# Hfx-J/SGTD

Hardware: AMD Instinct MI355X
Metric: query frames/sec vs map size (descriptor build + candidate selection) (higher is better)
Workload: dtype f64

## Files before the change

### sgtd_amd/csrc/build_kernel.hip.h

```cpp
#pragma once
#include "common.hip.h"

struct DescArrays {
  double *side, *angle, *center;
  float *vertex;
  int *label;
  u32 *frame;
  int *node_id;
  QueryRec *qrec;
};

#define SGTD_BUILD_THREADS 1024
#ifdef SGTD_EXP_PHASE
__device__ unsigned long long g_bphase[8];
#define BPH(i) do { if (tid == 0) { const unsigned long long _n = __builtin_readcyclecounter(); atomicAdd(&g_bphase[i], _n - bph_t); bph_t = _n; } } while (0)
#else
#define BPH(i) do { } while (0)
#endif
#define SGTD_TRI_INVALID 0xFFFFFFFFFFFFFFFFull
#define SGTD_SLOT_EMPTY 0xFFFFFFFFu

struct Tri {
  double a, b, c;
  int va, vb, vc;
  bool valid;
};

__device__ __forceinline__ double side_len(const float4 &p, const float4 &q) {
  double dx = (double)(p.x - q.x), dy = (double)(p.y - q.y), dz = (double)(p.z - q.z);
  return sqrt(dx * dx + dy * dy + dz * dz);
}

__device__ __forceinline__ Tri make_triangle(const float4 &p1, const float4 &p2,
                                             const float4 &p3, const DevCfg &cfg) {
  Tri t;
  double a = side_len(p1, p2), b = side_len(p1, p3), c = side_len(p3, p2);
  t.valid = !(a > cfg.max_len || b > cfg.max_len || c > cfg.max_len ||
              a < cfg.min_len || b < cfg.min_len || c < cfg.min_len);
  int sa = 0, sb = 1, sc = 2;
  double tmp; int ti;
  if (a > b) { tmp = a; a = b; b = tmp; ti = sa; sa = sb; sb = ti; }
  if (b > c) { tmp = b; b = c; c = tmp; ti = sb; sb = sc; sc = ti; }
  if (a > b) { tmp = a; a = b; b = tmp; ti = sa; sa = sb; sb = ti; }
  t.a = a; t.b = b; t.c = c;
  t.va = sa + sb - 1;
  t.vb = sa + sc - 1;
  t.vc = sb + sc - 1;
  return t;
}

__host__ __device__ __forceinline__ u64 pack_milli_key(u64 x, u64 y, u64 z) { return (x << 42) | (y << 21) | z; }
__device__ __forceinline__ u64 milli_key(const Tri &t) {
  float kx = (float)(t.a * 1000.0), ky = (float)(t.b * 1000.0), kz = (float)(t.c * 1000.0);
  u64 x = (u64)(long long)kx, y = (u64)(long long)ky, z = (u64)(long long)kz;
  return pack_milli_key(x, y, z);
}

struct BuildParams {
  const float *xyz;
  const u32 *label;
  const long long *kp_off;
  int n_frames;
  u32 frame_id0;
  int frame_id_step;
  long long out_stride;
  u32 *out_count;
  int max_n;
  int max_slots;
  u64 *ws_keys;
  u32 *ws_slots;
};

template <bool LDS_DEDUP, int KM>
__global__ __launch_bounds__(SGTD_BUILD_THREADS) void build_frames_kernel(
    BuildParams P, DevCfg cfg, DescArrays out) {
  extern __shared__ __align__(16) unsigned char smem[];
  const int K = cfg.K, tpi = cfg.tpi;
  const int max_t = P.max_n * tpi;
  const int max_words = (max_t + 31) / 32;
  float4 *pts = reinterpret_cast<float4 *>(smem);
  size_t off = (size_t)P.max_n * 16;
  unsigned short *knn = reinterpret_cast<unsigned short *>(smem + off);
  off += (((size_t)P.max_n * K * 2) + 15) & ~(size_t)15;
  unsigned char *mn = smem + off;
  off += (((size_t)tpi * 2) + 15) & ~(size_t)15;
  u32 *winbits = reinterpret_cast<u32 *>(smem + off);
  off += (((size_t)max_words * 4) + 15) & ~(size_t)15;
  u32 *wordpre = reinterpret_cast<u32 *>(smem + off);
  off += (((size_t)(max_words + 1) * 4) + 15) & ~(size_t)15;
  u64 *keys;
  u32 *slots;
  if (LDS_DEDUP) {
    keys = reinterpret_cast<u64 *>(smem + off);
    off += (size_t)max_t * 8;
    slots = reinterpret_cast<u32 *>(smem + off);
  } else {
    keys = P.ws_keys + (size_t)blockIdx.x * max_t;
    slots = P.ws_slots + (size_t)blockIdx.x * P.max_slots;
  }
  const int tid = threadIdx.x;

  if (tid == 0) {
    int k = 0;
    for (int m = 1; m < K - 1; m++)
      for (int n = m + 1; n < K; n++) {
        mn[2 * k] = (unsigned char)m;
        mn[2 * k + 1] = (unsigned char)n;
        k++;
      }
  }

  for (int f = blockIdx.x; f < P.n_frames; f += gridDim.x) {
    const long long kp0 = P.kp_off[f];
    const int n = (int)(P.kp_off[f + 1] - kp0);
    __syncthreads();
    if (n < K) {
      if (tid == 0) P.out_count[f] = 0;
      continue;
    }
    const int T = n * tpi;
    int nslots = 64;
    while (nslots < T + 1) nslots <<= 1;
    const int nwords = (T + 31) / 32;

#ifdef SGTD_EXP_PHASE
    unsigned long long bph_t = __builtin_readcyclecounter();
#endif
    for (int i = tid; i < n; i += SGTD_BUILD_THREADS) {
      float4 p;
      p.x = P.xyz[(kp0 + i) * 3 + 0];
      p.y = P.xyz[(kp0 + i) * 3 + 1];
      p.z = P.xyz[(kp0 + i) * 3 + 2];
      p.w = __uint_as_float(P.label[kp0 + i]);
      pts[i] = p;
    }
    for (int s = tid; s < nslots; s += SGTD_BUILD_THREADS) slots[s] = SGTD_SLOT_EMPTY;
    for (int w = tid; w < nwords; w += SGTD_BUILD_THREADS) winbits[w] = 0;
    __syncthreads();

    BPH(0);
    const int parts = (3 * K <= tpi) ? 4 : 1;
    const int per_pass = SGTD_BUILD_THREADS / parts;
    for (int i0 = 0; i0 < n; i0 += per_pass) {
      const int i = i0 + tid / parts, part = tid % parts;
      float bd[KM];
      int bi[KM];
#pragma unroll
      for (int k = 0; k < KM; k++) { bd[k] = __builtin_inff(); bi[k] = 0; }
      auto insert = [&](float cd, int cj) {
        bool lt = false;
#pragma unroll
        for (int k = 0; k < KM; k++) {
          lt = lt || (cd < bd[k]);
          float td = lt ? bd[k] : cd; int tj = lt ? bi[k] : cj;
          bd[k] = lt ? cd : bd[k]; bi[k] = lt ? cj : bi[k];
          cd = td; cj = tj;
        }
      };
      if (i < n) {
        const float4 q = pts[i];
        const int j_lo = (int)((long long)n * part / parts), j_hi = (int)((long long)n * (part + 1) / parts);
        for (int j = j_lo; j < j_hi; j++) {
          const float4 p = pts[j];
          float dx = q.x - p.x, dy = q.y - p.y, dz = q.z - p.z;
          float d = dx * dx;
          d += dy * dy;
          d += dz * dz;
          insert(d, j);
        }
        if (part > 0) {
#pragma unroll
          for (int k = 0; k < KM; k++)
            if (k < K) keys[((size_t)i * 3 + (part - 1)) * K + k] = ((u64)__float_as_uint(bd[k]) << 32) | (u32)bi[k];
        }
      }
      if (parts > 1) {
        if (!LDS_DEDUP) __threadfence_block();
        __syncthreads();
        if (i < n && part == 0) {
          for (int pk = 0; pk < 3 * K; pk++) {
            const u64 v = keys[(size_t)i * 3 * K + pk];
            insert(__uint_as_float((u32)(v >> 32)), (int)(u32)v);
          }
        }
      }
      if (i < n && part == 0) {
#pragma unroll
        for (int k = 0; k < KM; k++)
          if (k < K) knn[i * K + k] = (unsigned short)bi[k];
      }
      if (parts > 1) __syncthreads();
    }
    __syncthreads();

    BPH(1);
    for (int t = tid; t < T; t += SGTD_BUILD_THREADS) {
      const int i = t / tpi, r = t - i * tpi;
      const int m = mn[2 * r], nn = mn[2 * r + 1];
      Tri tr = make_triangle(pts[i], pts[knn[i * K + m]], pts[knn[i * K + nn]], cfg);
      keys[t] = tr.valid ? milli_key(tr) : SGTD_TRI_INVALID;
    }
    if (!LDS_DEDUP) __threadfence_block();
    __syncthreads();

    BPH(2);
    for (int t = tid; t < T; t += SGTD_BUILD_THREADS) {
      const u64 key = keys[t];
      if (key == SGTD_TRI_INVALID) continue;
      u32 h = (u32)mix64(key) & (u32)(nslots - 1);
      while (true) {
        u32 cur = atomicCAS(&slots[h], SGTD_SLOT_EMPTY, (u32)t);
        if (cur == SGTD_SLOT_EMPTY) break;
        if (keys[cur] == key) { atomicMin(&slots[h], (u32)t); break; }
        h = (h + 1) & (u32)(nslots - 1);
      }
    }
    __syncthreads();
    for (int s = tid; s < nslots; s += SGTD_BUILD_THREADS) {
      u32 v = slots[s];
      if (v != SGTD_SLOT_EMPTY) atomicOr(&winbits[v >> 5], 1u << (v & 31));
    }
    __syncthreads();
    if (tid < SGTD_WAVE) {
      u32 carry = 0;
      for (int w0 = 0; w0 < nwords; w0 += SGTD_WAVE) {
        int w = w0 + tid;
        u32 c = (w < nwords) ? __popc(winbits[w]) : 0;
        u32 inc = wave_incl_scan(c);
        if (w < nwords) wordpre[w] = carry + inc - c;
        carry += __shfl(inc, SGTD_WAVE - 1);
      }
      if (tid == 0) { wordpre[nwords] = carry; P.out_count[f] = carry; }
    }
    __syncthreads();

    BPH(3);
    const u32 frame_id = P.frame_id0 + (u32)(P.frame_id_step * f);
    for (int t = tid; t < T; t += SGTD_BUILD_THREADS) {
      const u32 word = winbits[t >> 5];
      if (!((word >> (t & 31)) & 1u)) continue;
      const u32 rank = wordpre[t >> 5] + __popc(word & ((1u << (t & 31)) - 1u));
      const int i = t / tpi, r = t - i * tpi;
      const int m = mn[2 * r], nn = mn[2 * r + 1];
      float4 p[3];
      p[0] = pts[i]; p[1] = pts[knn[i * K + m]]; p[2] = pts[knn[i * K + nn]];
      const Tri tr = make_triangle(p[0], p[1], p[2], cfg);
      const float4 A = tr.va == 0 ? p[0] : (tr.va == 1 ? p[1] : p[2]);
      const float4 B = tr.vb == 0 ? p[0] : (tr.vb == 1 ? p[1] : p[2]);
      const float4 C = tr.vc == 0 ? p[0] : (tr.vc == 1 ? p[1] : p[2]);
      const size_t o = (size_t)f * P.out_stride + rank;
      const double a = tr.a, b = tr.b, c = tr.c;
      out.side[o * 3 + 0] = cfg.scale * a;
      out.side[o * 3 + 1] = cfg.scale * b;
      out.side[o * 3 + 2] = cfg.scale * c;
      out.angle[o * 3 + 0] = fabs((b * b + c * c - a * a) / (2 * b * c));
      out.angle[o * 3 + 1] = fabs((a * a + c * c - b * b) / (2 * a * c));
      out.angle[o * 3 + 2] = fabs((a * a + b * b - c * c) / (2 * a * b));
      out.center[o * 3 + 0] = (((double)A.x + (double)B.x) + (double)C.x) / 3;
      out.center[o * 3 + 1] = (((double)A.y + (double)B.y) + (double)C.y) / 3;
      out.center[o * 3 + 2] = (((double)A.z + (double)B.z) + (double)C.z) / 3;
      out.vertex[o * 9 + 0] = A.x; out.vertex[o * 9 + 1] = A.y; out.vertex[o * 9 + 2] = A.z;
      out.vertex[o * 9 + 3] = B.x; out.vertex[o * 9 + 4] = B.y; out.vertex[o * 9 + 5] = B.z;
      out.vertex[o * 9 + 6] = C.x; out.vertex[o * 9 + 7] = C.y; out.vertex[o * 9 + 8] = C.z;
      out.label[o * 3 + 0] = (int)(double)__float_as_uint(A.w);
      out.label[o * 3 + 1] = (int)(double)__float_as_uint(B.w);
      out.label[o * 3 + 2] = (int)(double)__float_as_uint(C.w);
      out.frame[o] = frame_id;
      if (out.qrec) write_query_rec(out.qrec + o, cfg.scale * a, cfg.scale * b, cfg.scale * c, cfg.rough, frame_id);
      out.node_id[o * 3 + 0] = i; out.node_id[o * 3 + 1] = m; out.node_id[o * 3 + 2] = nn;
    }
#ifdef SGTD_EXP_PHASE
    __syncthreads();
    BPH(4);
#endif
  }
}

static inline size_t build_lds_bytes(int max_n, int K, int tpi, bool lds_dedup, int max_slots) {
  size_t max_t = (size_t)max_n * tpi, words = (max_t + 31) / 32;
  auto up = [](size_t v) { return (v + 15) & ~(size_t)15; };
  size_t b = (size_t)max_n * 16 + up((size_t)max_n * K * 2) + up((size_t)tpi * 2) +
             up(words * 4) + up((words + 1) * 4);
  if (lds_dedup) b += max_t * 8 + (size_t)max_slots * 4;
  return b;
}
```

### sgtd_amd/csrc/sgtd_accel.hip

```cpp
#include "../../include/sgtd_accel.h"

#include <hip/hip_runtime.h>

#include <algorithm>
#include <atomic>
#include <chrono>
#include <cmath>
#include <cstdio>
#include <cstring>
#include <limits>
#include <memory>
#include <string>
#include <vector>

#include "build_kernel.hip.h"
#include "common.hip.h"
#include "table_kernels.hip.h"
#include "probe_kernels.hip.h"
#include "select_kernels.hip.h"
#include "verify_kernels.hip.h"
#include "verify_mfma.hip.h"
#include "exchange_kernels.hip.h"
#include "remove_kernels.hip.h"
#include "filter_kernels.hip.h"
// ... 114 lines not shown
  };
  Segment seg[2];
  int n_seg = 1;
  u32 append_min_frame = 0xFFFFFFFFu;
  int64_t tail_max = 0;
  float ms_finalize = 0.f;
  u32 coarse_at = 62, whole_at = 62;
  long long thr2_pending = 0;
  u32 rec_rate_hook = 0;
  u32 rec_rate_cap = 256;
  bool wide_pairs = false;
  int tail_batches = 0;
  DevBuf slice_of, sq_sum;
  DevBuf frame_first, by_frame, id_of_g, longest;
  u32 id_bits = 0;
  bool id_by_frame = false;
  DevBuf rm_bits, rm_present, rm_mask, rm_count, rm_scratch;
  std::shared_ptr<const FrameFilter> filt, batch_filt;
  DevBuf filt_rows;
  std::vector<u64> filt_host;
  u64 filt_rows_serial = 0;
  u32 filt_rows_lo = 0, filt_rows_span = 0;
  std::vector<float> poses;
  std::vector<unsigned char> has_pose;
  u64 poses_serial = 0;
  std::shared_ptr<const PositionPrior> prior, batch_prior;
  DevBuf pos_dev, prior_dev, filt_base;
  std::vector<float4> pos_host;
  u64 pos_serial = 0;
  u32 pos_lo = 0, pos_span = 0;
  u64 filt_base_serial = 0;
  u32 filt_base_lo = 0, filt_base_span = 0;
  struct PriorKey {
    u64 prior = 0, poses = 0, filt = 0;
    u32 lo = 0, span = 0;
    int n_rows = 0;
    bool operator==(const PriorKey &o) const { return prior == o.prior && poses == o.poses && filt == o.filt && lo == o.lo && span == o.span && n_rows == o.n_rows; }
  } prior_key;
  bool prior_rows_valid = false;
  DevBuf keyA, keyB, valA, valB, hist, digit_tot, flags, bad_flag;
  std::vector<DevBuf> scan_lvl;

  DevBuf kp_off_dev, xyz_dev, label_dev, ws_keys, ws_slots, cnt_scan;
  DevBuf b_kp_off_dev, b_xyz_dev, b_label_dev;
  DescStore tmp;
  DescStore fetch;
  DevBuf fetch_idx;
  DevBuf tmp_count;

  DescStore qd;
  DevBuf q_count;
  long long q_stride = 0;
  int nq = 0;
  bool batch_valid = false, batch_synced = false;
  int last_kind = 0;
  const float *last_xyz = nullptr;
  const u32 *last_label = nullptr;
  std::vector<long long> last_kp_off;
  int last_max_n = 0;
  u32 last_qframe = 0;
  bool loop_batch = false;
  int loop_skip = 0;
  DevBuf totals;
  DevBuf cursors, list, n_visit, votes, slot_of;
  DevBuf q_M, q_P, q_pairs, q_pair_base, blk_count, rec, rec_cell, rec_dis;
  DevBuf c_pair, c_blk;
  DevBuf amb_queue;
  DevBuf n_cand, cand_frame, cand_votes, pair_off, pairs;
  DevBuf v_score, v_pose, v_inlier, v_best;
  DevBuf inl_pairs, inl_off;
  bool verify_counted = false;
  DevBuf inl_counts;
  DevBuf in_block;
  size_t frame_inl_cap = 0;
  char *frame_host = nullptr;
  size_t frame_host_bytes = 0;
  DevBuf b_in, b_out;
  char *pin_build = nullptr;
  size_t pin_build_cap = 0;
  DevBuf v_hyp64, v_hyp32, v_bound;
  DevBuf v_hypB, v_tau, v_words;
  DevBuf v_okey[2], v_oval[2];
  bool verified = false;
  DevBuf r_pose, r_rmse, r_rmse_v, r_npairs, r_moments, r_flag;
  bool refined = false;
  int *export_packed = nullptr;
  size_t export_cap = 0;
  hipEvent_t ev_cand = nullptr, ev_export_free = nullptr;
  bool export_busy = false;
  u32 batch_serial = 0;
  bool defer_lists = false;
  bool lists_pending = false;
  bool lists_masked = false;
  bool fused_votes_last = false;
  const u64 *verify_keep = nullptr;
  const u64 *list_keep = nullptr;
  bool pairs_per_query = false;
  DevBuf rough_qi, rough_entry, rough_frame, rough_cell, rough_dis;
  size_t rec_cap = (size_t)1 << 25;
  bool rec_cap_fixed = false;
  size_t pair_cap = (size_t)1 << 24;
  DevBuf n_valid, cell_rows, gid, q_prefix, group_first, n_groups;
  DevBuf pos_of_slot, rec_off, pass_pool;
  size_t pool_units = 0;
  size_t group_cap = 0;
  size_t group_cap_hook = 0;
  int sorted_chunk = 0;
  bool diag = false;
  int select_mode = 0;
  PinnedVec<u32> h_count, h_pair_base, h_q_M;
  PinnedVec<unsigned long long> h_q_P;
  PinnedVec<int> h_n_cand, h_cand_frame, h_cand_votes;
  PinnedVec<long long> h_pair_off;
  sgtd_stats stats{};
  char *pin = nullptr;
  size_t pin_cap = 0, pin_used = 0;
  struct PinCopy { void *dst; size_t off, bytes; };
  std::vector<PinCopy> pin_pending;
};

#include "multi.hip.h"

namespace {

#define HIPCHK(call)                                                          \
  do {                                                                        \
    hipError_t _s = (call);                                                   \
    if (_s != hipSuccess) {                                                   \
      e->err = std::string(#call) + ": " + hipGetErrorString(_s);             \
      return SGTD_ERR_HIP;                                                    \
    }                                                                         \
  } while (0)
#define CHK(call)                 \
  do {                            \
    int _r = (call);              \
    if (_r != SGTD_OK) return _r; \
  } while (0)

int ensure(sgtd_engine *e, DevBuf &b, size_t bytes, bool keep = false) {
  if (bytes <= b.bytes) return SGTD_OK;
  if (b.borrowed) { e->err = "a table attached from another handle cannot grow here"; return SGTD_ERR_STATE; }
  size_t want = keep ? std::max(bytes, b.bytes + b.bytes / 2) : (b.p ? bytes + bytes / 4 : bytes);
  if (!keep && b.p) {
    HIPCHK(hipStreamSynchronize(e->stream));
    HIPCHK(hipFree(b.p));
    b.p = nullptr; b.bytes = 0;
  }
  void *np = nullptr;
  {
    const hipError_t st_ = hipMalloc(&np, want);
    if (st_ != hipSuccess) {
      (void)hipGetLastError();
      e->err = "hipMalloc of " + std::to_string(want) + " bytes: " + hipGetErrorString(st_);
      return SGTD_ERR_HIP;
    }
  }
  e->stats.device_allocs_total++;
  if (keep && b.p && b.bytes) {
    HIPCHK(hipMemcpyAsync(np, b.p, b.bytes, hipMemcpyDeviceToDevice, e->stream));
    HIPCHK(hipStreamSynchronize(e->stream));
  }
  if (b.p) HIPCHK(hipFree(b.p));
  b.p = np;
  b.bytes = want;
  return SGTD_OK;
}

int ensure_store(sgtd_engine *e, DescStore &s, size_t cap, bool keep = false) {
  if (cap <= s.cap) return SGTD_OK;
  size_t want = keep ? std::max(cap, s.cap + s.cap / 2) : cap;
  CHK(ensure(e, s.side, want * 3 * sizeof(double), keep));
  CHK(ensure(e, s.angle, want * 3 * sizeof(double), keep));
  CHK(ensure(e, s.center, want * 3 * sizeof(double), keep));
  CHK(ensure(e, s.vertex, want * 9 * sizeof(float), keep));
  CHK(ensure(e, s.label, want * 3 * sizeof(int), keep));
  CHK(ensure(e, s.frame, want * sizeof(u32), keep));
  CHK(ensure(e, s.node_id, want * 3 * sizeof(int), keep));
  if (s.with_thr2) CHK(ensure(e, s.qrec, want * sizeof(QueryRec), keep));
  s.cap = want;
  return SGTD_OK;
}

void free_buf(DevBuf &b) {
  if (b.p && !b.borrowed) (void)hipFree(b.p);
  b.p = nullptr;
  b.bytes = 0;
  b.borrowed = false;
}
void free_store(DescStore &s) {
  free_buf(s.side); free_buf(s.angle); free_buf(s.center); free_buf(s.vertex);
  free_buf(s.label); free_buf(s.frame); free_buf(s.node_id); free_buf(s.qrec);
  s.cap = 0;
}

constexpr size_t kPinMax = (size_t)1 << 20, kPinCap = (size_t)16 << 20;

int xfer_sync(sgtd_engine *e) {
  HIPCHK(hipStreamSynchronize(e->stream));
  for (const auto &c : e->pin_pending) std::memcpy(c.dst, e->pin + c.off, c.bytes);
  e->pin_pending.clear();
  e->pin_used = 0;
  return SGTD_OK;
}

struct PinScope {
  sgtd_engine *e;
  explicit PinScope(sgtd_engine *e_) : e(e_) {}
  ~PinScope() {
    if (e && !e->pin_pending.empty()) {
      (void)hipStreamSynchronize(e->stream);
      e->pin_pending.clear();
      e->pin_used = 0;
    }
  }
};

int pin_room(sgtd_engine *e, size_t bytes, size_t *off) {
  if (!e->pin) {
    void *p = nullptr;
    HIPCHK(hipHostMalloc(&p, kPinCap, hipHostMallocDefault));
    e->pin = static_cast<char *>(p);
    e->pin_cap = kPinCap;
  }
  const size_t need = (bytes + 255) & ~(size_t)255;
  if (e->pin_used + need > e->pin_cap) CHK(xfer_sync(e));
  *off = e->pin_used;
  e->pin_used += need;
  return SGTD_OK;
}

int d2h(sgtd_engine *e, void *dst, const void *src_dev, size_t bytes) {
  if (bytes == 0) return SGTD_OK;
  if (bytes > kPinMax) {
    HIPCHK(hipMemcpyAsync(dst, src_dev, bytes, hipMemcpyDeviceToHost, e->stream));
    return SGTD_OK;
  }
  size_t off;
  CHK(pin_room(e, bytes, &off));
  HIPCHK(hipMemcpyAsync(e->pin + off, src_dev, bytes, hipMemcpyDeviceToHost, e->stream));
  e->pin_pending.push_back({dst, off, bytes});
  return SGTD_OK;
}

int h2d(sgtd_engine *e, void *dst_dev, const void *src, size_t bytes) {
  if (bytes == 0) return SGTD_OK;
  if (bytes > kPinMax) {
    HIPCHK(hipMemcpyAsync(dst_dev, src, bytes, hipMemcpyHostToDevice, e->stream));
    return SGTD_OK;
  }
  size_t off;
  CHK(pin_room(e, bytes, &off));
  std::memcpy(e->pin + off, src, bytes);
  HIPCHK(hipMemcpyAsync(dst_dev, e->pin + off, bytes, hipMemcpyHostToDevice, e->stream));
  return SGTD_OK;
}

int grid_for(long long n, int threads) { return (int)((n + threads - 1) / threads); }
constexpr size_t kIndexLimit = 0xFFFFFFF0ull;
constexpr size_t kRecLimit = kIndexLimit << SGTD_REC_SHIFT;
template <class K>
size_t lds_room(K *kernel) {
  hipFuncAttributes a;
  const size_t fixed = hipFuncGetAttributes(&a, reinterpret_cast<const void *>(kernel)) == hipSuccess ? a.sharedSizeBytes : 16384;
  return std::min<size_t>(150 * 1024, 160 * 1024 - std::min<size_t>(fixed, 160 * 1024));
}

int device_scan(sgtd_engine *e, const u32 *in, u32 *out, long long n, size_t lvl = 0) {
  if (n <= 0) return SGTD_OK;
  const long long per = (long long)SGTD_SCAN_THREADS * SGTD_SCAN_ITEMS;
  const long long nb = (n + per - 1) / per;
  if (nb == 1) {
    scan_apply_kernel<<<1, SGTD_SCAN_THREADS, 0, e->stream>>>(in, out, nullptr, n);
    HIPCHK(hipGetLastError());
    return SGTD_OK;
  }
  if (e->scan_lvl.size() <= lvl) e->scan_lvl.resize(lvl + 1);
  CHK(ensure(e, e->scan_lvl[lvl], (size_t)nb * sizeof(u32)));
  u32 *sums = e->scan_lvl[lvl].as<u32>();
  scan_reduce_kernel<<<(int)nb, SGTD_SCAN_THREADS, 0, e->stream>>>(in, sums, n);
  HIPCHK(hipGetLastError());
  CHK(device_scan(e, sums, sums, nb, lvl + 1));
  sums = e->scan_lvl[lvl].as<u32>();
  scan_apply_kernel<<<(int)nb, SGTD_SCAN_THREADS, 0, e->stream>>>(in, out, sums, n);
  HIPCHK(hipGetLastError());
  return SGTD_OK;
}

int launch_build(sgtd_engine *e, const float *d_xyz, const u32 *d_label, const long long *d_kp_off,
                 int n_frames, int max_n, u32 frame_id0, int frame_step, DescArrays out,
                 long long out_stride, u32 *out_count) {
  if (n_frames <= 0) return SGTD_OK;
  if (max_n > 65535) return SGTD_ERR_UNSUPPORTED;
  const int K = e->dc.K, tpi = e->dc.tpi;
  long long max_t = (long long)std::max(max_n, 1) * tpi;
  int max_slots = 64;
  while (max_slots < max_t + 1) max_slots <<= 1;
  const size_t lds_limit = 160 * 1024;
  size_t lds_full = build_lds_bytes(std::max(max_n, 1), K, tpi, true, max_slots);
  size_t lds_base = build_lds_bytes(std::max(max_n, 1), K, tpi, false, max_slots);
  BuildParams P;
  P.xyz = d_xyz; P.label = d_label; P.kp_off = d_kp_off; P.n_frames = n_frames;
  P.frame_id0 = frame_id0; P.frame_id_step = frame_step; P.out_stride = out_stride;
  P.out_count = out_count; P.max_n = std::max(max_n, 1); P.max_slots = max_slots;
  P.ws_keys = nullptr; P.ws_slots = nullptr;
  if (lds_full <= lds_limit) {
    int per_cu = (int)std::max<size_t>(1, lds_limit / lds_full);
    int grid = std::min(n_frames, e->n_cus * std::min(per_cu, 4));
#define SGTD_LAUNCH_BUILD(DEDUP, KM_, LDS_)                                                                    \
  do {                                                                                                          \
    HIPCHK(hipFuncSetAttribute(reinterpret_cast<const void *>(&build_frames_kernel<DEDUP, KM_>),                \
                               hipFuncAttributeMaxDynamicSharedMemorySize, (int)(LDS_)));                       \
    build_frames_kernel<DEDUP, KM_><<<grid, SGTD_BUILD_THREADS, (LDS_), e->stream>>>(P, e->dc, out);            \
  } while (0)
#define SGTD_LAUNCH_BUILD_K(DEDUP, LDS_)                                                                        \
  do {                                                                                                          \
    if (K <= 4) SGTD_LAUNCH_BUILD(DEDUP, 4, LDS_);                                                              \
    else if (K <= 8) SGTD_LAUNCH_BUILD(DEDUP, 8, LDS_);                                                         \
    else if (K <= 10) SGTD_LAUNCH_BUILD(DEDUP, 10, LDS_);                                                       \
    else if (K <= 12) SGTD_LAUNCH_BUILD(DEDUP, 12, LDS_);                                                       \
    else SGTD_LAUNCH_BUILD(DEDUP, 16, LDS_);                                                                    \
  } while (0)
    SGTD_LAUNCH_BUILD_K(true, lds_full);
  } else if (lds_base <= lds_limit) {
    int grid = std::min(n_frames, e->n_cus * 2);
    CHK(ensure(e, e->ws_keys, (size_t)grid * max_t * sizeof(u64)));
    CHK(ensure(e, e->ws_slots, (size_t)grid * max_slots * sizeof(u32)));
    P.ws_keys = e->ws_keys.as<u64>();
    P.ws_slots = e->ws_slots.as<u32>();
    SGTD_LAUNCH_BUILD_K(false, lds_base);
#undef SGTD_LAUNCH_BUILD_K
#undef SGTD_LAUNCH_BUILD
  } else {
    return SGTD_ERR_UNSUPPORTED;
  }
  HIPCHK(hipGetLastError());
  return SGTD_OK;
}

int stage_inputs(sgtd_engine *e, const float *xyz, const u32 *label, const int64_t *kp_off,
                 int n_frames, int device_ptrs, const float **d_xyz, const u32 **d_label,
                 int *max_n, bool own_set = false) {
  DevBuf &kp_buf = own_set ? e->b_kp_off_dev : e->kp_off_dev;
  DevBuf &xyz_buf = own_set ? e->b_xyz_dev : e->xyz_dev;
  DevBuf &label_buf = own_set ? e->b_label_dev : e->label_dev;
  std::vector<long long> off(n_frames + 1);
  int mx = 0;
  for (int f = 0; f <= n_frames; f++) off[f] = kp_off[f];
  for (int f = 0; f < n_frames; f++) {
    long long n = off[f + 1] - off[f];
    if (n < 0 || n > 65535) return SGTD_ERR_INVALID;
    mx = std::max(mx, (int)n);
  }
  *max_n = mx;
  CHK(ensure(e, kp_buf, (size_t)(n_frames + 1) * sizeof(long long)));
  if ((size_t)(n_frames + 1) * sizeof(long long) <= kPinMax) {
    CHK(h2d(e, kp_buf.p, off.data(), (size_t)(n_frames + 1) * sizeof(long long)));
  } else {
    HIPCHK(hipMemcpyAsync(kp_buf.p, off.data(), (size_t)(n_frames + 1) * sizeof(long long), hipMemcpyHostToDevice, e->stream));
    CHK(xfer_sync(e));
  }
  const long long total = off[n_frames] - off[0];
  if (device_ptrs) {
    *d_xyz = xyz;
    *d_label = label;
  } else {
    CHK(ensure(e, xyz_buf, (size_t)std::max<long long>(total + off[0], 1) * 3 * sizeof(float)));
    CHK(ensure(e, label_buf, (size_t)std::max<long long>(total + off[0], 1) * sizeof(u32)));
    if (total > 0) {
      CHK(h2d(e, xyz_buf.as<float>() + off[0] * 3, xyz + off[0] * 3,
                            (size_t)total * 3 * sizeof(float)));
      CHK(h2d(e, label_buf.as<u32>() + off[0], label + off[0], (size_t)total * sizeof(u32)));
    }
    *d_xyz = xyz_buf.as<float>();
    *d_label = label_buf.as<u32>();
  }
  return SGTD_OK;
}

int copy_out(sgtd_engine *e, const DescStore &s, size_t first, size_t n, sgtd_desc_soa *out, size_t dst0) {
  if (n == 0) return SGTD_OK;
#define CP(field, T, w)                                                                       \
  if (out->field)                                                                             \
    CHK(d2h(e, out->field + dst0 * (w), s.field.as<T>() + first * (w),             \
                          n * (w) * sizeof(T)));
  CP(side, double, 3) CP(angle, double, 3) CP(center, double, 3) CP(vertex, float, 9)
  CP(label, int, 3) CP(frame, u32, 1) CP(node_id, int, 3)
#undef CP
  CHK(xfer_sync(e));
  return SGTD_OK;
}

int copy_in(sgtd_engine *e, DescStore &s, size_t first, size_t n, const sgtd_desc_soa *in, bool wait = true) {
  if (n == 0) return SGTD_OK;
  const DescBlockOffsets bo = desc_block_offsets(n);
  static const bool block_on = [] { const char *o = getenv("SGTD_COPY_IN_BLOCK"); return !(o && !atoi(o)); }();
  if (block_on && bo.total <= (4u << 20)) {
    size_t off;
    CHK(pin_room(e, bo.total, &off));
    const void *src[7] = {in->side, in->angle, in->center, in->vertex, in->label, in->frame, in->node_id};
    void *dst[7] = {s.side.as<double>() + first * 3, s.angle.as<double>() + first * 3, s.center.as<double>() + first * 3, s.vertex.as<float>() + first * 9,
                    s.label.as<int>() + first * 3, s.frame.as<u32>() + first, s.node_id.as<int>() + first * 3};
    const size_t bytes[7] = {n * 24, n * 24, n * 24, n * 36, n * 12, n * 4, n * 12};
    u32 present = 0;
    for (int f = 0; f < 7; f++) {
      if (src[f]) { std::memcpy(e->pin + off + bo.off[f], src[f], bytes[f]); present |= 1u << f; }
      else HIPCHK(hipMemsetAsync(dst[f], 0, bytes[f], e->stream));
    }
    CHK(ensure(e, e->in_block, bo.total));
    HIPCHK(hipMemcpyAsync(e->in_block.p, e->pin + off, bo.total, hipMemcpyHostToDevice, e->stream));
    unpack_desc_block_kernel<<<(unsigned)std::min<long long>(grid_for((long long)n * 34, 256), 512), 256, 0, e->stream>>>(e->in_block.as<unsigned char>(), (u32)n, present, s.view(),
                                                                                                                       (long long)first);
    HIPCHK(hipGetLastError());
    if (wait) CHK(xfer_sync(e));
    return SGTD_OK;
  }
#define CP(field, T, w)                                                                        \
  if (in->field)                                                                               \
    CHK(h2d(e, s.field.as<T>() + first * (w), in->field, n * (w) * sizeof(T)));               \
  else                                                                                         \
    HIPCHK(hipMemsetAsync(s.field.as<T>() + first * (w), 0, n * (w) * sizeof(T), e->stream));
  CP(side, double, 3) CP(angle, double, 3) CP(center, double, 3) CP(vertex, float, 9)
  CP(label, int, 3) CP(frame, u32, 1) CP(node_id, int, 3)
#undef CP
  if (wait) CHK(xfer_sync(e));
  return SGTD_OK;
}

void note_frames(sgtd_engine *e, u32 lo, u32 hi) {
  if (!e->have_frames) {
    e->frame_lo = lo; e->frame_hi = hi; e->have_frames = true;
  } else {
    e->frame_lo = std::min(e->frame_lo, lo);
    e->frame_hi = std::max(e->frame_hi, hi);
  }
}

template <class KeyT>
int radix_sort_pairs(sgtd_engine *e, KeyT *&kin, KeyT *&kout, u32 *&vin, u32 *&vout, long long n, int bits,
                     bool skip_const, const u32 *n_dev = nullptr) {
  const int nblocks = (int)((n + SGTD_RS_TILE - 1) / SGTD_RS_TILE);
  CHK(ensure(e, e->hist, (size_t)256 * nblocks * sizeof(u32)));
  CHK(ensure(e, e->digit_tot, 256 * sizeof(u32)));
  std::vector<u32> tot(256);
  for (int shift = 0; shift < bits; shift += 8) {
    u32 *hist = e->hist.as<u32>();
    radix_hist_kernel<KeyT><<<nblocks, SGTD_RS_THREADS, 0, e->stream>>>(kin, n, shift, hist, nblocks, n_dev);
    HIPCHK(hipGetLastError());
    if (skip_const) {
      radix_digit_totals_kernel<<<256, SGTD_SCAN_THREADS, 0, e->stream>>>(hist, nblocks, e->digit_tot.as<u32>());
      HIPCHK(hipGetLastError());
      HIPCHK(hipMemcpyAsync(tot.data(), e->digit_tot.p, 256 * sizeof(u32), hipMemcpyDeviceToHost, e->stream));
      HIPCHK(hipStreamSynchronize(e->stream));
      bool constant = false;
      for (int d = 0; d < 256; d++)
        if ((long long)tot[d] == n) constant = true;
      if (constant) continue;
    }
    CHK(device_scan(e, hist, hist, (long long)256 * nblocks));
    radix_scatter_kernel<KeyT><<<nblocks, SGTD_RS_THREADS, 0, e->stream>>>(kin, vin, kout, vout, n, shift,
                                                                       e->hist.as<u32>(), nblocks, n_dev);
    HIPCHK(hipGetLastError());
    std::swap(kin, kout);
    std::swap(vin, vout);
  }
  return SGTD_OK;
}

IdMap id_map(const sgtd_engine *e, u32 bits) {
  IdMap m;
  m.frame_first = e->frame_first.as<u32>();
  m.by_frame = e->id_by_frame ? e->by_frame.as<u32>() : nullptr;
  m.bits = bits;
  m.frame_lo = e->have_frames ? e->frame_lo : 0;
  return m;
}

int build_segment(sgtd_engine *e, sgtd_engine::Segment &S, long long g0, long long g1) {
  const long long E = g1 - g0;
  S.g0 = g0; S.g1 = g1;
  S.n_buckets = 0;
  S.hash_mask = 1023;
  S.sum_len_sq = 0.0;
  S.frame_hi = e->have_frames ? e->frame_hi : 0;
  S.built = true;
  if (E == 0) {
    CHK(ensure(e, S.hash, (size_t)1024 * sizeof(HashSlot)));
    HIPCHK(hipMemsetAsync(S.hash.p, 0xFF, (size_t)1024 * sizeof(HashSlot), e->stream));
    return SGTD_OK;
  }
  const double *side = e->tab.side.as<double>() + (size_t)g0 * 3;
  const int *label = e->tab.label.as<int>() + (size_t)g0 * 3;
  const u32 *frame = e->tab.frame.as<u32>() + (size_t)g0;
  CHK(ensure(e, e->keyA, (size_t)E * sizeof(u64)));
  CHK(ensure(e, e->keyB, (size_t)E * sizeof(u64)));
  CHK(ensure(e, e->valA, (size_t)E * sizeof(u32)));
  CHK(ensure(e, e->valB, (size_t)E * sizeof(u32)));
  CHK(ensure(e, e->bad_flag, 2 * sizeof(int)));
  HIPCHK(hipMemsetAsync(e->bad_flag.p, 0, 2 * sizeof(int), e->stream));
  make_keys_kernel<<<grid_for(E, 256), 256, 0, e->stream>>>(side, label, e->keyA.as<u64>(), e->valA.as<u32>(), E,
                                                             e->bad_flag.as<int>());
  HIPCHK(hipGetLastError());
  frame_monotone_kernel<<<grid_for(E, 256), 256, 0, e->stream>>>(frame, E, e->bad_flag.as<int>() + 1);
  HIPCHK(hipGetLastError());
  int bad[2] = {0, 0};
  HIPCHK(hipMemcpyAsync(bad, e->bad_flag.p, sizeof(bad), hipMemcpyDeviceToHost, e->stream));
  HIPCHK(hipStreamSynchronize(e->stream));
  if (bad[0]) { S.built = false; return SGTD_ERR_UNSUPPORTED; }
  const bool monotone = bad[1] == 0;

  u64 *kin = e->keyA.as<u64>(), *kout = e->keyB.as<u64>();
  u32 *vin = e->valA.as<u32>(), *vout = e->valB.as<u32>();
  CHK(ensure(e, e->slice_of, (size_t)E));
  if (!monotone) {
    frame_keys_kernel<<<grid_for(E, 256), 256, 0, e->stream>>>(frame, kin, vin, E);
    HIPCHK(hipGetLastError());
    CHK(radix_sort_pairs(e, kin, kout, vin, vout, E, 32, true));
    keys_of_order_kernel<<<grid_for(E, 256), 256, 0, e->stream>>>(side, label, vin, kin, E);
    HIPCHK(hipGetLastError());
    CHK(radix_sort_pairs(e, kin, kout, vin, vout, E, 60, true));
    slice_assign_kernel<<<grid_for(E, 256), 256, 0, e->stream>>>(kin, vin, side, frame, E, e->dc.rough, e->slice_of.as<unsigned char>());
    HIPCHK(hipGetLastError());
    kin = e->keyA.as<u64>(); kout = e->keyB.as<u64>(); vin = e->valA.as<u32>(); vout = e->valB.as<u32>();
    make_keys_kernel<<<grid_for(E, 256), 256, 0, e->stream>>>(side, label, kin, vin, E, e->bad_flag.as<int>());
    HIPCHK(hipGetLastError());
  }
  CHK(radix_sort_pairs(e, kin, kout, vin, vout, E, 60, true));
  if (monotone) {
    slice_assign_kernel<<<grid_for(E, 256), 256, 0, e->stream>>>(kin, vin, side, frame, E, e->dc.rough, e->slice_of.as<unsigned char>());
    HIPCHK(hipGetLastError());
  }
  CHK(ensure(e, e->flags, (size_t)E * sizeof(u32)));
  head_flags_kernel<<<grid_for(E, 256), 256, 0, e->stream>>>(kin, e->flags.as<u32>(), E);
  HIPCHK(hipGetLastError());
  u32 last_flag = 0, last_excl = 0;
  HIPCHK(hipMemcpyAsync(&last_flag, e->flags.as<u32>() + (E - 1), sizeof(u32), hipMemcpyDeviceToHost, e->stream));
  CHK(device_scan(e, e->flags.as<u32>(), e->flags.as<u32>(), E));
  HIPCHK(hipMemcpyAsync(&last_excl, e->flags.as<u32>() + (E - 1), sizeof(u32), hipMemcpyDeviceToHost, e->stream));
  HIPCHK(hipStreamSynchronize(e->stream));
  const u32 U = last_excl + last_flag;
  S.n_buckets = U;
  CHK(ensure(e, S.bucket_start, (size_t)(U + 1) * sizeof(u32)));
  CHK(ensure(e, S.bucket_key, (size_t)U * sizeof(u64)));
  bucket_starts_kernel<<<grid_for(E, 256), 256, 0, e->stream>>>(kin, e->flags.as<u32>(), S.bucket_start.as<u32>(),
                                                                 S.bucket_key.as<u64>(), E);
  HIPCHK(hipGetLastError());
  CHK(ensure(e, S.perm, (size_t)(E + SGTD_SENTINELS) * sizeof(u32)));
  CHK(ensure(e, S.dir, (size_t)U * sizeof(BucketDir)));
  slice_partition_kernel<<<e->n_cus * 8, 256, 0, e->stream>>>(S.bucket_start.as<u32>(), U, (u32)E, vin,
                                                               e->slice_of.as<unsigned char>(), S.perm.as<u32>(),
                                                               S.dir.as<BucketDir>());
  HIPCHK(hipGetLastError());
  HotEntry *hot = nullptr;
  if (&S == &e->seg[1]) {
    sgtd_engine::Segment &M = e->seg[0];
    const size_t m_ent = (size_t)(M.g1 - M.g0) + SGTD_SENTINELS;
    CHK(ensure(e, M.hot, (m_ent + (size_t)E + SGTD_SENTINELS) * sizeof(HotEntry), true));
    hot = M.hot.as<HotEntry>() + m_ent;
  } else {
    const size_t tail_room = e->tail_max > 0 ? 0 : (size_t)std::max<long long>(262144, E / 8) + SGTD_SENTINELS;
    CHK(ensure(e, S.hot, ((size_t)(E + SGTD_SENTINELS) + tail_room) * sizeof(HotEntry)));
    hot = S.hot.as<HotEntry>();
  }
  gather_hot_kernel<<<grid_for(E + SGTD_SENTINELS, 256), 256, 0, e->stream>>>(
      S.perm.as<u32>(), side, frame, e->id_by_frame ? e->id_of_g.as<u32>() : nullptr, id_map(e, e->id_bits), hot, E, (u32)g0);
  HIPCHK(hipGetLastError());
  u32 cap = 1024;
  while (cap < 2ull * U) cap <<= 1;
  S.hash_mask = cap - 1;
  CHK(ensure(e, S.hash, (size_t)cap * sizeof(HashSlot)));
  HIPCHK(hipMemsetAsync(S.hash.p, 0xFF, (size_t)cap * sizeof(HashSlot), e->stream));
  hash_insert_kernel<<<grid_for(U, 256), 256, 0, e->stream>>>(S.bucket_key.as<u64>(), S.bucket_start.as<u32>(), U,
                                                               (u32)E, S.hash.as<HashSlot>(), S.hash_mask);
  HIPCHK(hipGetLastError());
  CHK(ensure(e, e->sq_sum, sizeof(unsigned long long)));
  HIPCHK(hipMemsetAsync(e->sq_sum.p, 0, sizeof(unsigned long long), e->stream));
  bucket_sq_kernel<<<grid_for(U, 256), 256, 0, e->stream>>>(S.bucket_start.as<u32>(), U, (u32)E, e->sq_sum.as<unsigned long long>());
  HIPCHK(hipGetLastError());
  unsigned long long sq = 0;
  HIPCHK(hipMemcpyAsync(&sq, e->sq_sum.p, sizeof(sq), hipMemcpyDeviceToHost, e->stream));
  HIPCHK(hipStreamSynchronize(e->stream));
  S.sum_len_sq = (double)sq;
  return SGTD_OK;
}

int build_idmap(sgtd_engine *e, u32 &bits) {
  const long long E = e->n_entries;
  bits = e->id_bits ? e->id_bits : 13;
  if (E == 0 || !e->have_frames) return SGTD_OK;
  const u32 lo = e->frame_lo, span = e->frame_hi - e->frame_lo + 1;
  const u32 *frame = e->tab.frame.as<u32>();
  CHK(ensure(e, e->frame_first, (size_t)span * sizeof(u32)));
  CHK(ensure(e, e->longest, 2 * sizeof(u32)));
  HIPCHK(hipMemsetAsync(e->longest.p, 0, 2 * sizeof(u32), e->stream));
  frame_monotone_kernel<<<grid_for(E, 256), 256, 0, e->stream>>>(frame, E, reinterpret_cast<int *>(e->longest.as<u32>() + 1));
  HIPCHK(hipGetLastError());
  u32 h[2] = {0, 0};
  HIPCHK(hipMemcpyAsync(h, e->longest.p, sizeof(h), hipMemcpyDeviceToHost, e->stream));
  HIPCHK(hipStreamSynchronize(e->stream));
  e->id_by_frame = h[1] != 0;
  const u32 *key = frame;
  if (e->id_by_frame) {
    CHK(ensure(e, e->keyA, (size_t)E * sizeof(u64)));
    CHK(ensure(e, e->keyB, (size_t)E * sizeof(u64)));
    CHK(ensure(e, e->valA, (size_t)E * sizeof(u32)));
    CHK(ensure(e, e->valB, (size_t)E * sizeof(u32)));
    u64 *kin = e->keyA.as<u64>(), *kout = e->keyB.as<u64>();
    u32 *vin = e->valA.as<u32>(), *vout = e->valB.as<u32>();
    frame_keys_kernel<<<grid_for(E, 256), 256, 0, e->stream>>>(frame, kin, vin, E);
    HIPCHK(hipGetLastError());
    CHK(radix_sort_pairs(e, kin, kout, vin, vout, E, 32, true));
    CHK(ensure(e, e->by_frame, (size_t)E * sizeof(u32)));
    CHK(ensure(e, e->id_of_g, (size_t)E * sizeof(u32)));
    HIPCHK(hipMemcpyAsync(e->by_frame.p, vin, (size_t)E * sizeof(u32), hipMemcpyDeviceToDevice, e->stream));
    low_words_kernel<<<grid_for(E, 256), 256, 0, e->stream>>>(kin, E, vout);
    HIPCHK(hipGetLastError());
    key = vout;
  }
  frame_first_kernel<<<grid_for(E, 256), 256, 0, e->stream>>>(key, E, lo, e->frame_first.as<u32>());
  HIPCHK(hipGetLastError());
  frame_longest_kernel<<<grid_for(E, 256), 256, 0, e->stream>>>(key, E, lo, e->frame_first.as<u32>(), e->longest.as<u32>());
  HIPCHK(hipGetLastError());
  HIPCHK(hipMemcpyAsync(h, e->longest.p, sizeof(u32), hipMemcpyDeviceToHost, e->stream));
  HIPCHK(hipStreamSynchronize(e->stream));
  u32 need = 1;
  while (need < 32 && (1ull << need) < (unsigned long long)h[0]) need++;
  auto fits = [&](u32 b) { return b < 32 && (unsigned long long)span < (1ull << (32 - b)) - 1ull; };
  if (bits < need || !fits(bits)) {
    bits = std::max<u32>(need, 13);
    if (!fits(bits)) bits = need;
    if (!fits(bits)) {
      e->err = "a 32-bit entry id cannot hold this table's frame span and its largest frame";
      return SGTD_ERR_UNSUPPORTED;
    }
  }
  if (e->id_by_frame) {
    id_of_sorted_kernel<<<grid_for(E, 256), 256, 0, e->stream>>>(key, e->by_frame.as<u32>(), E, lo, e->frame_first.as<u32>(), bits,
                                                                 e->id_of_g.as<u32>());
    HIPCHK(hipGetLastError());
// ... 2497 lines not shown
```

Measured before the change: 185,400.

## Stage descriptor fill through LDS for coalesced writes and merge KNN via DPP ranks

The output fill phase is reworked so each thread handles one winner, found by binary search over the per-word prefix counts. Each output array is first assembled in LDS in chunks, then copied to global memory with aligned 16-byte vector stores instead of scattered per-element writes. The cross-partition KNN merge now ranks candidates with DPP lane exchanges, replacing the spill to LDS, the extra barriers and the serial re-insertion. In exchange, the kernel needs more LDS, which can reduce blocks per CU, and adds many barriers per chunk.

```diff
diff --git a/sgtd_amd/csrc/build_kernel.hip.h b/sgtd_amd/csrc/build_kernel.hip.h
--- a/sgtd_amd/csrc/build_kernel.hip.h
+++ b/sgtd_amd/csrc/build_kernel.hip.h
@@ -17,6 +17,8 @@
 #else
 #define BPH(i) do { } while (0)
 #endif
+#define SGTD_FILL_CHUNK 1024
+#define SGTD_FILL_STAGE_BYTES (3 * (SGTD_FILL_CHUNK * 24 + 16))
 #define SGTD_TRI_INVALID 0xFFFFFFFFFFFFFFFFull
 #define SGTD_SLOT_EMPTY 0xFFFFFFFFu
 
@@ -56,6 +58,43 @@
   return pack_milli_key(x, y, z);
 }
 
+__device__ __forceinline__ int nth_winner(const u32 *winbits, const u32 *wordpre, int nwords, u32 r) {
+  int lo = 0, hi = nwords;
+  while (hi - lo > 1) {
+    const int mid = (lo + hi) >> 1;
+    if (wordpre[mid] <= r) lo = mid; else hi = mid;
+  }
+  const u32 bits = winbits[lo];
+  u32 k = r - wordpre[lo], pos = 0;
+#pragma unroll
+  for (u32 w = 16; w >= 1; w >>= 1) {
+    const u32 c = __popc((bits >> pos) & ((1u << w) - 1u));
+    if (k >= c) { k -= c; pos += w; }
+  }
+  return lo * 32 + (int)pos;
+}
+
+__device__ __forceinline__ unsigned char *fill_image(unsigned char *area, const void *dst) {
+  return area + ((size_t)dst & 15u);
+}
+
+__device__ __forceinline__ void lds_barrier() {
+  asm volatile("s_waitcnt lgkmcnt(0)\n\ts_barrier" ::: "memory");
+}
+
+__device__ __forceinline__ void fill_copy_out(const unsigned char *area, void *dst, u32 nbytes, int tid) {
+  const u32 lead = (u32)((size_t)dst & 15u), end = lead + nbytes;
+  unsigned char *g = reinterpret_cast<unsigned char *>(dst) - lead;
+  for (u32 b = (u32)tid * 16u; b < end; b += SGTD_BUILD_THREADS * 16u) {
+    if (b >= lead && b + 16u <= end) {
+      *reinterpret_cast<uint4 *>(g + b) = *reinterpret_cast<const uint4 *>(area + b);
+    } else {
+      const u32 w0 = b > lead ? b : lead, w1 = b + 16u < end ? b + 16u : end;
+      for (u32 w = w0; w < w1; w += 4u) *reinterpret_cast<u32 *>(g + w) = *reinterpret_cast<const u32 *>(area + w);
+    }
+  }
+}
+
 struct BuildParams {
   const float *xyz;
   const u32 *label;
@@ -67,6 +106,7 @@
   u32 *out_count;
   int max_n;
   int max_slots;
+  int staged_fill;
   u64 *ws_keys;
   u32 *ws_slots;
 };
@@ -168,28 +208,40 @@
           d += dz * dz;
           insert(d, j);
         }
-        if (part > 0) {
+      }
+#ifdef SGTD_EXP_PHASE
+      __syncthreads();
+      BPH(5);
+#endif
+      if (parts > 1) {
+        if (i < n) {
+          u32 rk[KM];
+#pragma unroll
+          for (int k = 0; k < KM; k++) rk[k] = (u32)k;
+#define SGTD_KNN_COUNT(CTRL, S)                                                                              \
+          {                                                                                                  \
+            const bool lower = part + (S) >= 4;    \
+            _Pragma("unroll") for (int j = 0; j < KM; j++) {                                                 \
+              if (j < K) {                                                                                   \
+                const u32 od = (u32)__builtin_amdgcn_update_dpp(0, (int)__float_as_uint(bd[j]), CTRL, 0xf, 0xf, false); \
+                const u32 odl = od + (lower ? 0u : 1u);    \
+                _Pragma("unroll") for (int k = 0; k < KM; k++) rk[k] += (__float_as_uint(bd[k]) >= odl) ? 1u : 0u; \
+              }                                                                                              \
+            }                                                                                                \
+          }
+          SGTD_KNN_COUNT(0x39, 1)
+          SGTD_KNN_COUNT(0x4E, 2)
+          SGTD_KNN_COUNT(0x93, 3)
+#undef SGTD_KNN_COUNT
 #pragma unroll
           for (int k = 0; k < KM; k++)
-            if (k < K) keys[((size_t)i * 3 + (part - 1)) * K + k] = ((u64)__float_as_uint(bd[k]) << 32) | (u32)bi[k];
-        }
-      }
-      if (parts > 1) {
-        if (!LDS_DEDUP) __threadfence_block();
-        __syncthreads();
-        if (i < n && part == 0) {
-          for (int pk = 0; pk < 3 * K; pk++) {
-            const u64 v = keys[(size_t)i * 3 * K + pk];
-            insert(__uint_as_float((u32)(v >> 32)), (int)(u32)v);
-          }
-        }
-      }
-      if (i < n && part == 0) {
+            if (k < K && rk[k] < (u32)K) knn[i * K + rk[k]] = (unsigned short)bi[k];
+        }
+      } else if (i < n) {
 #pragma unroll
         for (int k = 0; k < KM; k++)
           if (k < K) knn[i * K + k] = (unsigned short)bi[k];
       }
-      if (parts > 1) __syncthreads();
     }
     __syncthreads();
 
@@ -236,38 +288,103 @@
 
     BPH(3);
     const u32 frame_id = P.frame_id0 + (u32)(P.frame_id_step * f);
-    for (int t = tid; t < T; t += SGTD_BUILD_THREADS) {
-      const u32 word = winbits[t >> 5];
-      if (!((word >> (t & 31)) & 1u)) continue;
-      const u32 rank = wordpre[t >> 5] + __popc(word & ((1u << (t & 31)) - 1u));
+    struct Fill { double s[3], ang[3], cen[3]; float4 A, B, C; int i, m, nn; };
+    auto describe = [&](int t) {
+      Fill d;
       const int i = t / tpi, r = t - i * tpi;
       const int m = mn[2 * r], nn = mn[2 * r + 1];
       float4 p[3];
       p[0] = pts[i]; p[1] = pts[knn[i * K + m]]; p[2] = pts[knn[i * K + nn]];
       const Tri tr = make_triangle(p[0], p[1], p[2], cfg);
-      const float4 A = tr.va == 0 ? p[0] : (tr.va == 1 ? p[1] : p[2]);
-      const float4 B = tr.vb == 0 ? p[0] : (tr.vb == 1 ? p[1] : p[2]);
-      const float4 C = tr.vc == 0 ? p[0] : (tr.vc == 1 ? p[1] : p[2]);
-      const size_t o = (size_t)f * P.out_stride + rank;
+      d.A = tr.va == 0 ? p[0] : (tr.va == 1 ? p[1] : p[2]);
+      d.B = tr.vb == 0 ? p[0] : (tr.vb == 1 ? p[1] : p[2]);
+      d.C = tr.vc == 0 ? p[0] : (tr.vc == 1 ? p[1] : p[2]);
       const double a = tr.a, b = tr.b, c = tr.c;
-      out.side[o * 3 + 0] = cfg.scale * a;
-      out.side[o * 3 + 1] = cfg.scale * b;
-      out.side[o * 3 + 2] = cfg.scale * c;
-      out.angle[o * 3 + 0] = fabs((b * b + c * c - a * a) / (2 * b * c));
-      out.angle[o * 3 + 1] = fabs((a * a + c * c - b * b) / (2 * a * c));
-      out.angle[o * 3 + 2] = fabs((a * a + b * b - c * c) / (2 * a * b));
-      out.center[o * 3 + 0] = (((double)A.x + (double)B.x) + (double)C.x) / 3;
-      out.center[o * 3 + 1] = (((double)A.y + (double)B.y) + (double)C.y) / 3;
-      out.center[o * 3 + 2] = (((double)A.z + (double)B.z) + (double)C.z) / 3;
-      out.vertex[o * 9 + 0] = A.x; out.vertex[o * 9 + 1] = A.y; out.vertex[o * 9 + 2] = A.z;
-      out.vertex[o * 9 + 3] = B.x; out.vertex[o * 9 + 4] = B.y; out.vertex[o * 9 + 5] = B.z;
-      out.vertex[o * 9 + 6] = C.x; out.vertex[o * 9 + 7] = C.y; out.vertex[o * 9 + 8] = C.z;
-      out.label[o * 3 + 0] = (int)(double)__float_as_uint(A.w);
-      out.label[o * 3 + 1] = (int)(double)__float_as_uint(B.w);
-      out.label[o * 3 + 2] = (int)(double)__float_as_uint(C.w);
-      out.frame[o] = frame_id;
-      if (out.qrec) write_query_rec(out.qrec + o, cfg.scale * a, cfg.scale * b, cfg.scale * c, cfg.rough, frame_id);
-      out.node_id[o * 3 + 0] = i; out.node_id[o * 3 + 1] = m; out.node_id[o * 3 + 2] = nn;
+      d.s[0] = cfg.scale * a; d.s[1] = cfg.scale * b; d.s[2] = cfg.scale * c;
+      d.ang[0] = fabs((b * b + c * c - a * a) / (2 * b * c));
+      d.ang[1] = fabs((a * a + c * c - b * b) / (2 * a * c));
+      d.ang[2] = fabs((a * a + b * b - c * c) / (2 * a * b));
+      d.cen[0] = (((double)d.A.x + (double)d.B.x) + (double)d.C.x) / 3;
+      d.cen[1] = (((double)d.A.y + (double)d.B.y) + (double)d.C.y) / 3;
+      d.cen[2] = (((double)d.A.z + (double)d.B.z) + (double)d.C.z) / 3;
+      d.i = i; d.m = m; d.nn = nn;
+      return d;
+    };
+    if (LDS_DEDUP && P.staged_fill) {
+      unsigned char *const area0 = reinterpret_cast<unsigned char *>(keys);
+      const u32 count = wordpre[nwords];
+      for (u32 r0 = 0; r0 < count; r0 += SGTD_FILL_CHUNK) {
+        const u32 cnt = count - r0 < SGTD_FILL_CHUNK ? count - r0 : SGTD_FILL_CHUNK;
+        const size_t o0 = (size_t)f * P.out_stride + r0;
+        const bool act = (u32)tid < cnt;
+        Fill d;
+        if (act) d = describe(nth_winner(winbits, wordpre, nwords, r0 + (u32)tid));
+        {
+          unsigned char *const a_side = area0, *const a_angle = a_side + SGTD_FILL_CHUNK * 24 + 16,
+                              *const a_center = a_angle + SGTD_FILL_CHUNK * 24 + 16;
+          if (act) {
+            double *side = reinterpret_cast<double *>(fill_image(a_side, out.side + o0 * 3)) + tid * 3;
+            double *angle = reinterpret_cast<double *>(fill_image(a_angle, out.angle + o0 * 3)) + tid * 3;
+            double *center = reinterpret_cast<double *>(fill_image(a_center, out.center + o0 * 3)) + tid * 3;
+#pragma unroll
+            for (int k = 0; k < 3; k++) { side[k] = d.s[k]; angle[k] = d.ang[k]; center[k] = d.cen[k]; }
+          }
+          lds_barrier();
+          fill_copy_out(a_side, out.side + o0 * 3, cnt * 24u, tid);
+          fill_copy_out(a_angle, out.angle + o0 * 3, cnt * 24u, tid);
+          fill_copy_out(a_center, out.center + o0 * 3, cnt * 24u, tid);
+          lds_barrier();
+        }
+        {
+          unsigned char *const a_vertex = area0, *const a_label = a_vertex + SGTD_FILL_CHUNK * 36 + 16,
+                              *const a_node = a_label + SGTD_FILL_CHUNK * 12 + 16, *const a_frame = a_node + SGTD_FILL_CHUNK * 12 + 16;
+          if (act) {
+            float *vertex = reinterpret_cast<float *>(fill_image(a_vertex, out.vertex + o0 * 9)) + tid * 9;
+            int *label = reinterpret_cast<int *>(fill_image(a_label, out.label + o0 * 3)) + tid * 3;
+            int *node = reinterpret_cast<int *>(fill_image(a_node, out.node_id + o0 * 3)) + tid * 3;
+            u32 *frame = reinterpret_cast<u32 *>(fill_image(a_frame, out.frame + o0)) + tid;
+            vertex[0] = d.A.x; vertex[1] = d.A.y; vertex[2] = d.A.z;
+            vertex[3] = d.B.x; vertex[4] = d.B.y; vertex[5] = d.B.z;
+            vertex[6] = d.C.x; vertex[7] = d.C.y; vertex[8] = d.C.z;
+            label[0] = (int)(double)__float_as_uint(d.A.w);
+            label[1] = (int)(double)__float_as_uint(d.B.w);
+            label[2] = (int)(double)__float_as_uint(d.C.w);
+            node[0] = d.i; node[1] = d.m; node[2] = d.nn;
+            *frame = frame_id;
+          }
+          lds_barrier();
+          fill_copy_out(a_vertex, out.vertex + o0 * 9, cnt * 36u, tid);
+          fill_copy_out(a_label, out.label + o0 * 3, cnt * 12u, tid);
+          fill_copy_out(a_node, out.node_id + o0 * 3, cnt * 12u, tid);
+          fill_copy_out(a_frame, out.frame + o0, cnt * 4u, tid);
+          lds_barrier();
+        }
+        if (out.qrec) {
+          if (act) write_query_rec(reinterpret_cast<QueryRec *>(area0) + tid, d.s[0], d.s[1], d.s[2], cfg.rough, frame_id);
+          lds_barrier();
+          fill_copy_out(area0, out.qrec + o0, cnt * 64u, tid);
+          lds_barrier();
+        }
+      }
+    } else {
+      for (int t = tid; t < T; t += SGTD_BUILD_THREADS) {
+        const u32 word = winbits[t >> 5];
+        if (!((word >> (t & 31)) & 1u)) continue;
+        const u32 rank = wordpre[t >> 5] + __popc(word & ((1u << (t & 31)) - 1u));
+        const Fill d = describe(t);
+        const size_t o = (size_t)f * P.out_stride + rank;
+#pragma unroll
+        for (int k = 0; k < 3; k++) { out.side[o * 3 + k] = d.s[k]; out.angle[o * 3 + k] = d.ang[k]; out.center[o * 3 + k] = d.cen[k]; }
+        out.vertex[o * 9 + 0] = d.A.x; out.vertex[o * 9 + 1] = d.A.y; out.vertex[o * 9 + 2] = d.A.z;
+        out.vertex[o * 9 + 3] = d.B.x; out.vertex[o * 9 + 4] = d.B.y; out.vertex[o * 9 + 5] = d.B.z;
+        out.vertex[o * 9 + 6] = d.C.x; out.vertex[o * 9 + 7] = d.C.y; out.vertex[o * 9 + 8] = d.C.z;
+        out.label[o * 3 + 0] = (int)(double)__float_as_uint(d.A.w);
+        out.label[o * 3 + 1] = (int)(double)__float_as_uint(d.B.w);
+        out.label[o * 3 + 2] = (int)(double)__float_as_uint(d.C.w);
+        out.frame[o] = frame_id;
+        if (out.qrec) write_query_rec(out.qrec + o, d.s[0], d.s[1], d.s[2], cfg.rough, frame_id);
+        out.node_id[o * 3 + 0] = d.i; out.node_id[o * 3 + 1] = d.m; out.node_id[o * 3 + 2] = d.nn;
+      }
     }
 #ifdef SGTD_EXP_PHASE
     __syncthreads();
@@ -284,3 +401,8 @@
   if (lds_dedup) b += max_t * 8 + (size_t)max_slots * 4;
   return b;
 }
+
+static inline size_t build_lds_bytes_staged(int max_n, int K, int tpi, int max_slots) {
+  const size_t tables = (size_t)max_n * tpi * 8 + (size_t)max_slots * 4;
+  return build_lds_bytes(max_n, K, tpi, false, max_slots) + (tables > SGTD_FILL_STAGE_BYTES ? tables : (size_t)SGTD_FILL_STAGE_BYTES);
+}
diff --git a/sgtd_amd/csrc/sgtd_accel.hip b/sgtd_amd/csrc/sgtd_accel.hip
--- a/sgtd_amd/csrc/sgtd_accel.hip
+++ b/sgtd_amd/csrc/sgtd_accel.hip
@@ -440,8 +440,10 @@
   P.xyz = d_xyz; P.label = d_label; P.kp_off = d_kp_off; P.n_frames = n_frames;
   P.frame_id0 = frame_id0; P.frame_id_step = frame_step; P.out_stride = out_stride;
   P.out_count = out_count; P.max_n = std::max(max_n, 1); P.max_slots = max_slots;
-  P.ws_keys = nullptr; P.ws_slots = nullptr;
+  P.ws_keys = nullptr; P.ws_slots = nullptr; P.staged_fill = 0;
   if (lds_full <= lds_limit) {
+    const size_t lds_staged = build_lds_bytes_staged(std::max(max_n, 1), K, tpi, max_slots);
+    if (lds_staged <= lds_limit) { P.staged_fill = 1; lds_full = lds_staged; }
     int per_cu = (int)std::max<size_t>(1, lds_limit / lds_full);
     int grid = std::min(n_frames, e->n_cus * std::min(per_cu, 4));
 #define SGTD_LAUNCH_BUILD(DEDUP, KM_, LDS_)                                                                    \
@@ -472,6 +474,18 @@
     return SGTD_ERR_UNSUPPORTED;
   }
   HIPCHK(hipGetLastError());
+#ifdef SGTD_EXP_PHASE
+  if (n_frames >= 256) {
+    static unsigned long long prev[8];
+    unsigned long long ph[8];
+    HIPCHK(hipStreamSynchronize(e->stream));
+    HIPCHK(hipMemcpyFromSymbol(ph, HIP_SYMBOL(g_bphase), sizeof(ph)));
+    double d[8], tot = 0;
+    for (int k = 0; k < 8; k++) { d[k] = (double)(ph[k] - prev[k]); prev[k] = ph[k]; tot += d[k]; }
+    fprintf(stderr, "BPHASE frames %d (%.0f cycles a frame): load %.4f knn-scan %.4f knn-merge %.4f keys %.4f dedup+compact %.4f fill %.4f\n",
+            n_frames, tot / n_frames, d[0] / tot, d[5] / tot, d[1] / tot, d[2] / tot, d[3] / tot, d[4] / tot);
+  }
+#endif
   return SGTD_OK;
 }
 
```

Measured after the change: 182,400. 0.984x the previous value.
